# sec-bit/ckb-zkp

Measured on AMD Instinct MI355X. Metric: Groth16 proofs/sec (2^20 constraints, BN256), higher is better.
Workload: dtype u32 limbs (256-bit Montgomery integers); 1 GPU; Groth16 prove, MiMC-chain R1CS, 1048570 constraints (domain 2^20), 1258284 aux, bn254, G1 x4 + G2 x1 MSM + 4 NTT (7 in the reference: evaluation-form key); curve=bn254, log_domain=20, parallelism=independent proofs x1

## Files before the change

### ckb_zkp_amd/csrc/ctx.hpp

```cpp
#pragma once
#include <hip/hip_runtime.h>
#include <stdint.h>

#include <map>
#include <mutex>
#include <memory>
#include <string>
#include <unordered_map>
#include <vector>

#include "../../include/zkp_accel.h"

namespace zkp {

struct HipError {
  hipError_t e;
  const char* what;
  int line;
};

#define ZKP_HIP(call)                                                   \
  do {                                                                  \
    hipError_t _e = (call);                                             \
    if (_e != hipSuccess) throw ::zkp::HipError{_e, #call, __LINE__};   \
  } while (0)

struct StatusError {
  int32_t status;
};
#define ZKP_REQUIRE(cond, status) \
  do {                            \
    if (!(cond)) throw ::zkp::StatusError{(status)}; \
  } while (0)

struct DevBuf {
  void* p = nullptr;
  size_t cap = 0;
  void* get(size_t bytes) {
    if (bytes > cap) {
      if (p) (void)hipFree(p);
      p = nullptr;
      cap = 0;
      size_t want = bytes + (bytes >> 3) + 256;
      hipError_t e = hipMalloc(&p, want);
      if (e != hipSuccess) throw StatusError{ZKP_ERR_OOM};
      cap = want;
    }
    return p;
  }
  template <class T>
  T* as(size_t count) { return reinterpret_cast<T*>(get(count * sizeof(T))); }
  ~DevBuf() {
    if (p) (void)hipFree(p);
  }
  DevBuf() = default;
  DevBuf(const DevBuf&) = delete;
  DevBuf& operator=(const DevBuf&) = delete;
};

struct NttTables {
  int log_n = 0, h = 0;
  uint32_t* w_lo = nullptr;
  uint32_t* w_hi = nullptr;
  uint32_t* wi_lo = nullptr;
  uint32_t* wi_hi = nullptr;
  uint32_t* g_lo = nullptr;
  uint32_t* g_hi = nullptr;
  uint32_t* gi_lo = nullptr;
  uint32_t* gi_hi = nullptr;
  uint32_t* sub_fwd = nullptr;
  uint32_t* sub_inv = nullptr;
  uint32_t* n_inv = nullptr;
  void* block = nullptr;
  uint32_t* full_fwd[8] = {};
  uint32_t* full_inv[8] = {};
  uint32_t* full_g = nullptr;
  uint32_t* full_gi = nullptr;
  uint32_t* g_hi_n = nullptr;
  uint32_t* full_g_n = nullptr;
  std::vector<void*> extra;
};

struct BasesEntry;

struct MsmWorkspace {
  hipStream_t stream = nullptr;
  bool own_stream = false;
  hipEvent_t done = nullptr;
  hipEvent_t sorted = nullptr;
  hipEvent_t l1_done = nullptr;
  uint32_t chain_nb = 0;
  size_t chain_xb = 0;
  hipEvent_t acc_done = nullptr;
  DevBuf keys, vals, keys2, vals2, sort_tmp, offsets, buckets, tmp, out, sched, scan_tmp, scan_tmp2, partial, redo;
};
struct Groth16Timing {
  zkp_groth16_timing t{};
};

}

struct zkp_lane {
  hipStream_t stream = nullptr;
  bool own_stream = true;
  static constexpr int N_WS = 4;
  static constexpr int N_WS_MSM = N_WS;
  zkp::MsmWorkspace ws[N_WS];
  zkp::DevBuf ntt_scratch;
  hipEvent_t ev_fork = nullptr, ev_a = nullptr, ev_b1 = nullptr;
  uint32_t* host_proof = nullptr;
  bool host_tail = false;
  bool busy = false;
};

struct zkp_cfg {
  int lanes = 0;
  int msm_batch_lanes = 1;
  int msm_c = 0, msm_c_g2 = 0;
  long long msm_chunk = (long long)3 << 19;
  double table_budget_gb = 0;
  bool h_lagrange = true, c_fold = true, host_affine = true;
  long long lfold_heavy_cost = 0;
  int multi_exchange = 0;
  int multi_exchange_timeout_ms = 30000;
  int multi_wm_split = -1;
};

struct zkp_ctx {
  int device = 0;
  zkp_cfg cfg;
  std::recursive_mutex mu;
  static constexpr int N_LANES = 8;
  static constexpr int N_WS = zkp_lane::N_WS;
  zkp_lane lanes[N_LANES];
  zkp_lane* cur = &lanes[0];
  int cur_idx = 0;
  hipEvent_t ev0 = nullptr, ev1 = nullptr;
  hipEvent_t ev2 = nullptr, ev3 = nullptr;
  bool profiling = false;
  size_t table_bytes = 0;
  bool msm_defer_reduce = false;
  int msm_acc_into = -1;
  int msm_bucket_ws = -1;
  bool dbg_skip_k8 = false;
  bool batch_mode = false;
  std::map<std::pair<int, int>, zkp::NttTables> ntt_tables;
  zkp::DevBuf ntt_io, poly_tmp, poly_consts, spmv_list;
  zkp::DevBuf msm_scalars, msm_misc, var_bases;
  uint32_t* pinned = nullptr;
  size_t pinned_cap = 0;
  std::unordered_map<uint64_t, std::shared_ptr<zkp::BasesEntry>> bases;
  uint64_t next_handle = 1;
  zkp_groth16_timing last_timing{};
  zkp_marlin_timing last_marlin_timing{};
  std::string last_error;
  std::vector<zkp_ctx*> devs;
  std::map<std::pair<int, int>, std::shared_ptr<void>> var_plans;
  bool tl_on = false;
  std::string tl_tag;
  std::vector<std::pair<std::string, hipEvent_t>> tl;
  void mark(hipStream_t st, const char* what) {
    if (!tl_on) return;
    hipEvent_t e = nullptr;
    if (hipEventCreate(&e) != hipSuccess) return;
    (void)hipEventRecord(e, st);
    tl.emplace_back(tl_tag + what, e);
  }
};
```

### ckb_zkp_amd/csrc/groth16.hip

```cpp
#include <algorithm>
#include <cstdlib>
#include <cstring>
#include <memory>
#include <string>
#include <vector>

#include "field_dev.hpp"
#include "host_field.hpp"
#include "internal.hpp"
#include "msm_vtbl.hpp"

using namespace zkp;

struct DevCsr {
  uint32_t* row_ptr = nullptr;
  uint32_t* col = nullptr;
  uint32_t* coeff = nullptr;
  size_t nnz = 0;
};

struct zkp_groth16_pk {
  int curve = 0;
  uint32_t num_inputs = 0, num_aux = 0, num_constraints = 0;
  int log_n = 0;
// ... 502 lines not shown
        bases_set_sort_flags(ctx, pk->hA, all.data(), all.size());
        bases_set_group(ctx, pk->hA, member.data(), member.size());
        bases_set_filter_bit(ctx, pk->hA, 0);
        if (with_b) bases_set_filter_bit(ctx, pk->hB2, 1);
        bases_set_filter_bit(ctx, pk->hL, 2);
        pk->share_l1 = true;
        pk->b_in_l1 = with_b;
      }
      {
        static const bool on_chain = !(getenv("ZKP_CHAIN_LH") && atoi(getenv("ZKP_CHAIN_LH")) == 0);
        uint64_t iL[5], iH[5];
        bases_info(ctx, pk->hL, iL);
        bases_info(ctx, pk->hH, iH);
        pk->chain_lh = on_chain && iL[0] == iH[0] && iL[2] == 1 && iH[2] == 1 && pk->q_n[3] > 0 && pk->q_n[4] > 0;
      }
      if (getenv("ZKP_DEBUG_MSM"))
        fprintf(stderr, "[groth16] A/L sort sharing: %d (flags differ at %zu of %zu bases), B1/B2: %d, shared level 1: %d\n",
                (int)pk->share_al_sort, differ, fA.size(), (int)pk->share_b_sort, (int)pk->share_l1);
    }
  }
  uint32_t* consts = pk->consts.as<uint32_t>(64);
  if (d->curve == ZKP_BN254) hipLaunchKernelGGL(qap_consts_kernel<Bn254Fr>, dim3(1), dim3(64), 0, ctx->cur->stream, consts, lg);
  else hipLaunchKernelGGL(qap_consts_kernel<Bls381Fr>, dim3(1), dim3(64), 0, ctx->cur->stream, consts, lg);
  ZKP_HIP(hipGetLastError());
  for (int l = 0; l < 2; l++) {
    auto& L = pk->lane[l];
    L.abc.get(3 * pk->N * 32);
    L.S.get((pk->nz + 4) * 32);
    L.results.get(6 * 16 * 24 * 4 + 64);
    L.proof.get(4096);
  }
  ZKP_HIP(hipStreamSynchronize(ctx->cur->stream));
  return pk.release();
}

void groth16_pk_free(zkp_ctx* ctx, zkp_groth16_pk* pk) {
  (void)hipDeviceSynchronize();
  for (auto& PL : pk->lane) {
    if (PL.graph_exec) (void)hipGraphExecDestroy(PL.graph_exec);
    if (PL.graph) (void)hipGraphDestroy(PL.graph);
  }
  for (uint64_t h : {pk->hA, pk->hB1, pk->hB2, pk->hH, pk->hL})
    if (h) bases_drop(ctx, h);
  for (auto& m : pk->m) {
    if (m.row_ptr) (void)hipFree(m.row_ptr);
    if (m.col) (void)hipFree(m.col);
    if (m.coeff) (void)hipFree(m.coeff);
  }
  delete pk;
}

uint64_t groth16_domain_size(zkp_groth16_pk* pk) { return pk->N; }
void groth16_pk_info(zkp_ctx* ctx, zkp_groth16_pk* pk, uint64_t info[8]) {
  for (int i = 0; i < 8; i++) info[i] = 0;
  if (!pk->hA) return;
  uint64_t a[5], b[5];
  bases_info(ctx, pk->hA, a);
  bases_info(ctx, pk->hB2, b);
  info[0] = a[2];
  for (uint64_t h : {pk->hA, pk->hB1, pk->hB2, pk->hH, pk->hL}) {
    uint64_t t[5];
    bases_info(ctx, h, t);
    info[1] += t[4];
  }
  info[2] = a[0];
  info[3] = a[1];
  info[4] = a[3];
  info[5] = b[0];
  info[6] = (pk->share_b_sort ? 1 : 0) | (pk->share_al_sort ? 2 : 0) | (pk->share_l1 ? 4 : 0);
  info[7] = (pk->h_lagrange ? 1 : 0) | (pk->c_folded ? 2 : 0) | (pk->chain_lh ? 4 : 0);
}

template <class P>
static uint32_t* witness_map_dev(zkp_ctx* ctx, zkp_groth16_pk* pk, const uint32_t* z_dev, bool coeffs = true) {
  const uint32_t N = (uint32_t)pk->N;
  uint32_t* a = pk->lane[ctx->cur_idx].abc.as<uint32_t>(3 * pk->N * 8);
  uint32_t* b = a + pk->N * 8;
  uint32_t* c = b + pk->N * 8;
  uint32_t* bufs[3] = {a, b, c};
  hipStream_t st = ctx->cur->stream;
  const int nchain = (!coeffs && pk->c_folded) ? 2 : 3;
  for (int k = 0; k < nchain; k++)
    hipLaunchKernelGGL(csr_eval_kernel<P>, dim3((N + 255) / 256), dim3(256), 0, st, pk->m[k].row_ptr, pk->m[k].col,
                       pk->m[k].coeff, z_dev, pk->num_constraints, N, pk->num_inputs, k == 0 ? 1 : 0, bufs[k]);
  static const bool batch = getenv("ZKP_NTT_BATCH") && atoi(getenv("ZKP_NTT_BATCH")) != 0;
  if (batch) {
    ntt_run_batch(ctx, pk->curve, bufs, nchain, pk->log_n, ZKP_NTT_IFFT);
    ntt_run_batch(ctx, pk->curve, bufs, nchain, pk->log_n, ZKP_NTT_COSET_FFT);
  } else {
    for (int k = 0; k < nchain; k++) {
      if (!ntt_ifft_coset_fft(ctx, pk->curve, bufs[k], pk->log_n)) {
        ntt_run(ctx, pk->curve, bufs[k], pk->log_n, ZKP_NTT_IFFT);
        ntt_run(ctx, pk->curve, bufs[k], pk->log_n, ZKP_NTT_COSET_FFT);
      }
    }
  }
  if (!coeffs) {
    if (pk->c_folded) hipLaunchKernelGGL(qap_pointwise_ab_kernel<P>, dim3((N + 255) / 256), dim3(256), 0, st, a, b, pk->consts.as<uint32_t>(64), N);
    else hipLaunchKernelGGL(qap_pointwise_kernel<P>, dim3((N + 255) / 256), dim3(256), 0, st, a, b, c, pk->consts.as<uint32_t>(64), N);
    ZKP_HIP(hipGetLastError());
    return a;
  }
  if (uint32_t* hq = ntt_qap_coset_ifft(ctx, pk->curve, a, b, c, pk->consts.as<uint32_t>(64), pk->log_n)) {
    ZKP_HIP(hipGetLastError());
    return hq;
  }
  hipLaunchKernelGGL(qap_pointwise_kernel<P>, dim3((N + 255) / 256), dim3(256), 0, st, a, b, c,
                     pk->consts.as<uint32_t>(64), N);
  ntt_run(ctx, pk->curve, a, pk->log_n, ZKP_NTT_COSET_IFFT);
  ZKP_HIP(hipGetLastError());
  return a;
}

void groth16_witness_map(zkp_ctx* ctx, zkp_groth16_pk* pk, const uint64_t* z, uint64_t* h, bool on_device) {
  const uint32_t* zd = reinterpret_cast<const uint32_t*>(z);
  if (!on_device) {
    uint32_t* s = pk->lane[ctx->cur_idx].S.as<uint32_t>((pk->nz + 4) * 8);
    ZKP_HIP(hipMemcpyAsync(s, z, pk->nz * 32, hipMemcpyHostToDevice, ctx->cur->stream));
    zd = s;
  }
  uint32_t* hd = pk->curve == ZKP_BN254 ? witness_map_dev<Bn254Fr>(ctx, pk, zd) : witness_map_dev<Bls381Fr>(ctx, pk, zd);
  ZKP_HIP(hipMemcpyAsync(h, hd, pk->N * 32, on_device ? hipMemcpyDeviceToDevice : hipMemcpyDeviceToHost, ctx->cur->stream));
  if (!on_device) ZKP_HIP(hipStreamSynchronize(ctx->cur->stream));
}

template <class FrP>
static void prove_enqueue_part(zkp_ctx* ctx, zkp_groth16_pk* pk, const uint64_t* z, bool z_on_device, const uint64_t* r,
                               const uint64_t* s, int part, char* partial_out = nullptr, bool latency_plan = false) {
  ZKP_REQUIRE((pk->shard_world > 0) == (partial_out != nullptr), ZKP_ERR_BAD_ARG);
  ZKP_REQUIRE(pk->hA != 0, ZKP_ERR_BAD_ARG);
  zkp_groth16_pk::PerLane& PL = pk->lane[ctx->cur_idx];
  hipStream_t st = ctx->cur->stream;
  const bool prof = ctx->profiling;
  const bool host_tail = ctx->cfg.host_affine && !partial_out;
  zkp_groth16_timing tm{};
  struct ProfEvents {
    hipEvent_t e[4] = {nullptr, nullptr, nullptr, nullptr};
    ~ProfEvents() {
      for (hipEvent_t x : e)
        if (x) (void)hipEventDestroy(x);
    }
  } pev;
  if (prof)
    for (hipEvent_t& x : pev.e) ZKP_HIP(hipEventCreate(&x));
  hipEvent_t &e0 = pev.e[0], &e1 = pev.e[1], &eT0 = pev.e[2], &eT1 = pev.e[3];
  auto tic = [&] { if (prof) ZKP_HIP(hipEventRecord(e0, st)); };
  auto toc = [&](float* dst) {
    if (!prof) return;
    ZKP_HIP(hipEventRecord(e1, st));
    ZKP_HIP(hipEventSynchronize(e1));
    ZKP_HIP(hipEventElapsedTime(dst, e0, e1));
  };
  if (prof) ZKP_HIP(hipEventRecord(eT0, st));
  uint32_t* S = PL.S.as<uint32_t>((pk->nz + 4) * 8);
  uint32_t* rs = PL.proof.as<uint32_t>(1024);
  uint32_t* proof_dev = rs + 16;
  uint32_t* flags_dev = proof_dev + 256;
  if (part & 1) {
    ZKP_HIP(hipMemcpyAsync(S, z, pk->nz * 32, z_on_device ? hipMemcpyDeviceToDevice : hipMemcpyHostToDevice, st));
    ZKP_HIP(hipMemcpyAsync(rs, r, 32, hipMemcpyHostToDevice, st));
    ZKP_HIP(hipMemcpyAsync(rs + 8, s, 32, hipMemcpyHostToDevice, st));
  }
  if (!(part & 2)) return;
  hipLaunchKernelGGL(scalar_tail_kernel<FrP>, dim3(1), dim3(64), 0, st, S + pk->nz * 8, rs);

  const MsmVtbl* v1 = msm_vtbl(pk->curve, 1);
  const MsmVtbl* v2 = msm_vtbl(pk->curve, 2);
  const size_t slot = v2->xyzz_bytes;
  char* res = reinterpret_cast<char*>(PL.results.get(6 * slot));
  const uint64_t* Sd = reinterpret_cast<const uint64_t*>(S);
  bool l_done_in_fan = false, g2_done_in_fan = false, chained = false;
  float acc_ms = 0.f, scan_ms = 0.f;
  uint64_t ent = 0, scan_bytes = 0, scan_runs = 0;
  static const bool single_stream = getenv("ZKP_SINGLE_STREAM") && atoi(getenv("ZKP_SINGLE_STREAM")) != 0;
  const bool fan = !prof && !single_stream;
  uint32_t* h = nullptr;
  auto run = [&](int idx, uint64_t handle, const uint64_t* sc, size_t n, int w, int sort_src = -1, int l1_src = -1) {
    float ms = 0.f, ms_sc = 0.f;
    uint64_t e = 0;
    static const char* const names[5] = {"A", "B1", "B2", "H", "L"};
    ctx->tl_tag = names[idx];
    tic();
#ifdef ZKP_ABLATION
    static const int skip_k8 = [] { const char* e = getenv("ZKP_DEBUG_SKIP_K8_MASK"); return e ? (int)strtol(e, nullptr, 0) : 0; }();
    ctx->dbg_skip_k8 = ((skip_k8 >> idx) & 1) && ctx->batch_mode;
#endif
    msm_run(ctx, handle, 0, sc, n, true, nullptr, res + idx * slot, prof ? &ms : nullptr, &e, fan ? w : 0,
            fan ? sort_src : -1, prof ? &ms_sc : nullptr, fan ? l1_src : -1);
    ctx->dbg_skip_k8 = false;
    toc(&tm.ms_msm[idx]);
    acc_ms += ms;
    ent += e;
    tm.ms_msm_acc[idx] = ms;
    tm.msm_entries[idx] = e;
    if (ms_sc > 0.f) {
      scan_ms += ms_sc;
      scan_bytes += 2 * 32 * (uint64_t)n + 8 * e;
      scan_runs += 1;
    }
    tm.msm_accumulate_launches += 1;
  };
  ctx->tl_tag.clear();
  ctx->mark(st, "start");
  if (fan) {
    ZKP_HIP(hipEventRecord(ctx->cur->ev_fork, st));
    for (int w = 1; w < zkp_ctx::N_WS; w++) ZKP_HIP(hipStreamWaitEvent(ctx->cur->ws[w].stream, ctx->cur->ev_fork, 0));
    static const bool wm_first = !(getenv("ZKP_WM_FIRST") && atoi(getenv("ZKP_WM_FIRST")) == 0);
    if (wm_first) {
      h = witness_map_dev<FrP>(ctx, pk, S, !pk->h_lagrange);
      ctx->mark(st, "wm");
    }
    static const bool l_own = !(getenv("ZKP_L_OWN_STREAM") && atoi(getenv("ZKP_L_OWN_STREAM")) == 0);
    static const int lat_env = [] { const char* e = getenv("ZKP_LATENCY_PLAN"); return e ? atoi(e) : -1; }();
    (void)latency_plan;
    const bool lat = lat_env >= 0 ? lat_env != 0 : true;
    if (lat) {
      const int l1 = pk->share_l1 ? 1 : -1;
      const bool b_l1 = pk->share_l1 && pk->b_in_l1;
      if (!b_l1) run(2, pk->hB2, Sd + 4 * pk->q_lo[2], pk->q_n[2], 2);
      run(0, pk->hA, Sd + 4 * pk->q_lo[0], pk->q_n[0], 1);
      ZKP_HIP(hipEventRecord(ctx->cur->ev_a, ctx->cur->ws[1].stream));
      if (b_l1) run(2, pk->hB2, Sd + 4 * pk->q_lo[2], pk->q_n[2], 2, -1, l1);
      static const bool g2_early = !(getenv("ZKP_G2_EARLY") && atoi(getenv("ZKP_G2_EARLY")) == 0);
      if (!partial_out && g2_early && !host_tail) {
        v2->assemble_g2(ctx->cur->ws[2].stream, res, slot, proof_dev, flags_dev, 2 * v1->fN);
        g2_done_in_fan = true;
      }
      run(1, pk->hB1, Sd + 4 * pk->q_lo[1], pk->q_n[1], 3, pk->share_b_sort ? 2 : -1);
      ctx->msm_defer_reduce = chained = pk->chain_lh;
      run(4, pk->hL, Sd + 4 * pk->q_lo[4], pk->q_n[4], 1, pk->share_al_sort ? 1 : -1, l1);
      if (!partial_out) {
        ZKP_HIP(hipStreamWaitEvent(ctx->cur->ws[3].stream, ctx->cur->ev_a, 0));
        v1->assemble_g1_part1(ctx->cur->ws[3].stream, res, slot, rs, host_tail ? nullptr : proof_dev, flags_dev);
        ctx->tl_tag.clear();
        ctx->mark(ctx->cur->ws[3].stream, "part1");
      }
    } else {
    run(2, pk->hB2, Sd + 4 * pk->q_lo[2], pk->q_n[2], 2);
    run(0, pk->hA, Sd + 4 * pk->q_lo[0], pk->q_n[0], 1);
    run(1, pk->hB1, Sd + 4 * pk->q_lo[1], pk->q_n[1], 1, pk->share_b_sort ? 2 : -1);
    if (l_own) run(4, pk->hL, Sd + 4 * pk->q_lo[4], pk->q_n[4], 3, pk->share_al_sort && pk->share_b_sort ? 1 : -1);
    ZKP_HIP(hipEventRecord(ctx->cur->ev_b1, ctx->cur->ws[1].stream));
    if (!partial_out) {
      ZKP_HIP(hipStreamWaitEvent(ctx->cur->ws[3].stream, ctx->cur->ev_b1, 0));
      v1->assemble_g1_part1(ctx->cur->ws[3].stream, res, slot, rs, host_tail ? nullptr : proof_dev, flags_dev);
    }
    }
    l_done_in_fan = lat || l_own;
  }
  tic();
  if (!h) h = witness_map_dev<FrP>(ctx, pk, S, !pk->h_lagrange);
  toc(&tm.ms_witness_map);
  if (!fan) {
    run(0, pk->hA, Sd + 4 * pk->q_lo[0], pk->q_n[0], 0);
    run(1, pk->hB1, Sd + 4 * pk->q_lo[1], pk->q_n[1], 0);
    run(2, pk->hB2, Sd + 4 * pk->q_lo[2], pk->q_n[2], 0);
  }
  if (chained) ctx->msm_acc_into = 1;
  run(3, pk->hH, reinterpret_cast<const uint64_t*>(h) + 4 * pk->q_lo[3], pk->q_n[3], 0);
  if (!(fan && l_done_in_fan)) run(4, pk->hL, Sd + 4 * pk->q_lo[4], pk->q_n[4], 0);
  if (fan) {
    for (int w = 1; w < zkp_ctx::N_WS; w++) {
      ZKP_HIP(hipEventRecord(ctx->cur->ws[w].done, ctx->cur->ws[w].stream));
      ZKP_HIP(hipStreamWaitEvent(st, ctx->cur->ws[w].done, 0));
    }
  }
  tm.ms_msm_accumulate = acc_ms;
  tm.msm_points = ent;
  tm.ms_msm_scan = scan_ms;
  tm.msm_scan_bytes = scan_bytes;
  tm.msm_scan_launches = scan_runs;
  if (partial_out) {
    ZKP_HIP(hipMemcpyAsync(partial_out, res, 5 * slot, hipMemcpyDeviceToDevice, st));
    ZKP_HIP(hipGetLastError());
    if (prof) {
      ZKP_HIP(hipEventRecord(eT1, st));
      ZKP_HIP(hipStreamSynchronize(st));
      ZKP_HIP(hipEventElapsedTime(&tm.ms_total, eT0, eT1));
      ctx->last_timing = tm;
    }
    return;
  }

  tic();
  if (!fan) v1->assemble_g1_part1(st, res, slot, rs, host_tail ? nullptr : proof_dev, flags_dev);
  v1->assemble_g1_part2(st, res, slot, host_tail ? nullptr : proof_dev, flags_dev, 2 * v1->fN + 2 * v2->fN);
  if (!g2_done_in_fan && !host_tail) v2->assemble_g2(st, res, slot, proof_dev, flags_dev, 2 * v1->fN);
  ZKP_HIP(hipGetLastError());
  toc(&tm.ms_assemble);
  const size_t proof_words = 4 * (size_t)v1->fN + 2 * (size_t)v2->fN;
  if (host_tail) {
    uint32_t* hp = ctx->cur->host_proof;
    ZKP_HIP(hipMemcpyAsync(hp, res, 16 * (size_t)v1->fN, hipMemcpyDeviceToHost, st));
    ZKP_HIP(hipMemcpyAsync(hp + 4 * v1->fN, res + 2 * slot, 16 * (size_t)v2->fN, hipMemcpyDeviceToHost, st));
    ZKP_HIP(hipMemcpyAsync(hp + 4 * v1->fN + 4 * v2->fN, res + 5 * slot, 16 * (size_t)v1->fN, hipMemcpyDeviceToHost, st));
  } else {
    ZKP_HIP(hipMemcpyAsync(ctx->cur->host_proof, proof_dev, proof_words * 4, hipMemcpyDeviceToHost, st));
    ZKP_HIP(hipMemcpyAsync(ctx->cur->host_proof + 256, flags_dev, 12, hipMemcpyDeviceToHost, st));
  }
  ctx->tl_tag.clear();
  ctx->mark(st, "copied");
  ctx->cur->host_tail = host_tail;
  ctx->cur->busy = true;
  if (prof) {
    ZKP_HIP(hipEventRecord(eT1, st));
    ZKP_HIP(hipStreamSynchronize(st));
    ZKP_HIP(hipEventElapsedTime(&tm.ms_total, eT0, eT1));
    ctx->last_timing = tm;
  }
}

static std::vector<const void*> lane_signature(zkp_ctx* ctx, zkp_groth16_pk* pk) {
  std::vector<const void*> sig;
  zkp_lane* L = ctx->cur;
  zkp_groth16_pk::PerLane& PL = pk->lane[ctx->cur_idx];
  for (DevBuf* b : {&PL.abc, &PL.S, &PL.results, &PL.proof, &L->ntt_scratch}) sig.push_back(b->p);
  for (int w = 0; w < zkp_lane::N_WS; w++) {
    MsmWorkspace& ws = L->ws[w];
    for (DevBuf* b : {&ws.keys, &ws.vals, &ws.keys2, &ws.vals2, &ws.sort_tmp, &ws.offsets, &ws.buckets, &ws.tmp, &ws.out,
                      &ws.sched, &ws.scan_tmp, &ws.scan_tmp2, &ws.partial, &ws.redo})
      sig.push_back(b->p);
  }
  sig.push_back(pk);
  return sig;
}

template <class FrP>
static void prove_enqueue(zkp_ctx* ctx, zkp_groth16_pk* pk, const uint64_t* z, bool z_on_device, const uint64_t* r,
                          const uint64_t* s, bool latency_plan = false) {
  static const bool graph_on = getenv("ZKP_GRAPH") && atoi(getenv("ZKP_GRAPH")) != 0;
  static const bool single_stream = getenv("ZKP_SINGLE_STREAM") && atoi(getenv("ZKP_SINGLE_STREAM")) != 0;
  if (!graph_on || ctx->profiling || single_stream) {
    prove_enqueue_part<FrP>(ctx, pk, z, z_on_device, r, s, 3, nullptr, latency_plan);
    return;
  }
  zkp_groth16_pk::PerLane& PL = pk->lane[ctx->cur_idx];
  hipStream_t st = ctx->cur->stream;
  if (PL.graph_state == 2 && PL.sig == lane_signature(ctx, pk)) {
    prove_enqueue_part<FrP>(ctx, pk, z, z_on_device, r, s, 1);
    ZKP_HIP(hipGraphLaunch(PL.graph_exec, st));
    ctx->cur->busy = true;
    return;
  }
  if (PL.graph_state == 2) {
    (void)hipGraphExecDestroy(PL.graph_exec);
    (void)hipGraphDestroy(PL.graph);
    PL.graph_exec = nullptr;
    PL.graph = nullptr;
    PL.graph_state = 0;
  }
  if (PL.graph_state == 1 && PL.sig == lane_signature(ctx, pk)) {
    prove_enqueue_part<FrP>(ctx, pk, z, z_on_device, r, s, 1);
    ZKP_HIP(hipStreamBeginCapture(st, hipStreamCaptureModeRelaxed));
    try {
      prove_enqueue_part<FrP>(ctx, pk, z, z_on_device, r, s, 2);
    } catch (...) {
      hipGraph_t g = nullptr;
      (void)hipStreamEndCapture(st, &g);
      if (g) (void)hipGraphDestroy(g);
      throw;
    }
    ZKP_HIP(hipStreamEndCapture(st, &PL.graph));
    ZKP_HIP(hipGraphInstantiate(&PL.graph_exec, PL.graph, nullptr, nullptr, 0));
    PL.graph_state = 2;
    ZKP_HIP(hipGraphLaunch(PL.graph_exec, st));
    ctx->cur->busy = true;
    return;
  }
  prove_enqueue_part<FrP>(ctx, pk, z, z_on_device, r, s, 3);
  PL.sig = lane_signature(ctx, pk);
  PL.graph_state = 1;
}

static void prove_finish(zkp_ctx* ctx, zkp_groth16_pk* pk, uint64_t* proof_out, uint8_t* inf_out) {
  const MsmVtbl* v1 = msm_vtbl(pk->curve, 1);
  const MsmVtbl* v2 = msm_vtbl(pk->curve, 2);
  const size_t proof_words = 4 * (size_t)v1->fN + 2 * (size_t)v2->fN;
  ZKP_HIP(hipStreamSynchronize(ctx->cur->stream));
  if (!ctx->tl.empty()) {
    std::string line = "[zkp timeline ms]";
    for (auto& m : ctx->tl) {
      float ms = 0.f;
      (void)hipEventSynchronize(m.second);
      (void)hipEventElapsedTime(&ms, ctx->tl[0].second, m.second);
      char buf[64];
      snprintf(buf, sizeof buf, " %s=%.2f", m.first.c_str(), ms);
      line += buf;
      if (&m != &ctx->tl[0]) (void)hipEventDestroy(m.second);
    }
    (void)hipEventDestroy(ctx->tl[0].second);
    ctx->tl.clear();
    fprintf(stderr, "%s\n", line.c_str());
  }
  if (ctx->cur->host_tail) {
    const hostf::HostField Fq = hostf::fq_field(pk->curve);
    const uint32_t* hp = ctx->cur->host_proof;
    hostf::groth16_points_into_affine(Fq, hp, hp + 4 * v1->fN, hp + 4 * v1->fN + 4 * v2->fN,
                                      reinterpret_cast<uint32_t*>(proof_out), inf_out);
  } else {
    memcpy(proof_out, ctx->cur->host_proof, proof_words * 4);
    for (int i = 0; i < 3; i++) inf_out[i] = (uint8_t)ctx->cur->host_proof[256 + i];
  }
  ctx->cur->busy = false;
}

void groth16_assemble(zkp_ctx* ctx, int curve, const uint64_t* sums, const uint64_t* r, const uint64_t* s,
                      uint64_t* proof_out, uint8_t* inf_out) {
  const MsmVtbl* v1 = msm_vtbl(curve, 1);
  const MsmVtbl* v2 = msm_vtbl(curve, 2);
  hipStream_t st = ctx->cur->stream;
  const size_t slot = v2->xyzz_bytes;
  const size_t j1 = 3 * (size_t)v1->fN, j2 = 3 * (size_t)v2->fN;
  const size_t in_words = 4 * j1 + j2;
  uint32_t* buf = ctx->msm_misc.as<uint32_t>(in_words + 16 + 6 * slot / 4 + 256 + 16);
  uint32_t* jac = buf;
  uint32_t* rs = jac + in_words;
  char* res = reinterpret_cast<char*>(rs + 16);
  uint32_t* proof_dev = reinterpret_cast<uint32_t*>(res + 6 * slot);
  uint32_t* flags_dev = proof_dev + 240;
  ZKP_HIP(hipMemcpyAsync(jac, sums, in_words * 4, hipMemcpyHostToDevice, st));
  ZKP_HIP(hipMemcpyAsync(rs, r, 32, hipMemcpyHostToDevice, st));
  ZKP_HIP(hipMemcpyAsync(rs + 8, s, 32, hipMemcpyHostToDevice, st));
  const size_t off[5] = {0, j1, 2 * j1, 2 * j1 + j2, 3 * j1 + j2};
  for (int i = 0; i < 5; i++) (i == 2 ? v2 : v1)->from_jacobian(st, jac + off[i], res + i * slot);
  v1->assemble_g1_part1(st, res, slot, rs, proof_dev, flags_dev);
  v1->assemble_g1_part2(st, res, slot, proof_dev, flags_dev, 2 * v1->fN + 2 * v2->fN);
  v2->assemble_g2(st, res, slot, proof_dev, flags_dev, 2 * v1->fN);
  ZKP_HIP(hipGetLastError());
  const size_t proof_words = 4 * (size_t)v1->fN + 2 * (size_t)v2->fN;
  uint32_t flags_host[4] = {0, 0, 0, 0};
  ZKP_HIP(hipMemcpyAsync(proof_out, proof_dev, proof_words * 4, hipMemcpyDeviceToHost, st));
  ZKP_HIP(hipMemcpyAsync(flags_host, flags_dev, 12, hipMemcpyDeviceToHost, st));
  ZKP_HIP(hipStreamSynchronize(st));
  for (int i = 0; i < 3; i++) inf_out[i] = (uint8_t)flags_host[i];
}

size_t groth16_partials_bytes(int curve) { return 5 * msm_vtbl(curve, 2)->xyzz_bytes; }

void groth16_prove_partials(zkp_ctx* ctx, zkp_groth16_pk* pk, const uint64_t* z_dev, const uint64_t* r, const uint64_t* s,
                            void* out_dev) {
  ZKP_REQUIRE(pk->shard_world > 0, ZKP_ERR_BAD_ARG);
  ctx->cur = &ctx->lanes[0];
  ctx->cur_idx = 0;
  if (pk->curve == ZKP_BN254) prove_enqueue_part<Bn254Fr>(ctx, pk, z_dev, true, r, s, 3, (char*)out_dev, true);
  else prove_enqueue_part<Bls381Fr>(ctx, pk, z_dev, true, r, s, 3, (char*)out_dev, true);
  ZKP_HIP(hipStreamSynchronize(ctx->cur->stream));
}

void groth16_fold_assemble(zkp_ctx* ctx, int curve, const void* gathered_dev, int world, const uint64_t* r,
                           const uint64_t* s, uint64_t* proof_out, uint8_t* inf_out) {
  ZKP_REQUIRE(world >= 1, ZKP_ERR_BAD_ARG);
  const MsmVtbl* v1 = msm_vtbl(curve, 1);
  const MsmVtbl* v2 = msm_vtbl(curve, 2);
  hipStream_t st = ctx->cur->stream;
  const size_t slot = v2->xyzz_bytes;
  uint32_t* buf = ctx->msm_misc.as<uint32_t>(16 + 6 * slot / 4 + 256 + 16);
  uint32_t* rs = buf;
  char* res = reinterpret_cast<char*>(rs + 16);
  uint32_t* proof_dev = reinterpret_cast<uint32_t*>(res + 6 * slot);
  uint32_t* flags_dev = proof_dev + 240;
  ZKP_HIP(hipMemcpyAsync(rs, r, 32, hipMemcpyHostToDevice, st));
  ZKP_HIP(hipMemcpyAsync(rs + 8, s, 32, hipMemcpyHostToDevice, st));
  v1->fold_slots(st, (const char*)gathered_dev, 5 * slot, world, slot, 0x1b, res);
  v2->fold_slots(st, (const char*)gathered_dev, 5 * slot, world, slot, 0x04, res);
  v1->assemble_g1_part1(st, res, slot, rs, proof_dev, flags_dev);
  v1->assemble_g1_part2(st, res, slot, proof_dev, flags_dev, 2 * v1->fN + 2 * v2->fN);
  v2->assemble_g2(st, res, slot, proof_dev, flags_dev, 2 * v1->fN);
  ZKP_HIP(hipGetLastError());
  const size_t proof_words = 4 * (size_t)v1->fN + 2 * (size_t)v2->fN;
  uint32_t flags_host[4] = {0, 0, 0, 0};
  ZKP_HIP(hipMemcpyAsync(proof_out, proof_dev, proof_words * 4, hipMemcpyDeviceToHost, st));
  ZKP_HIP(hipMemcpyAsync(flags_host, flags_dev, 12, hipMemcpyDeviceToHost, st));
  ZKP_HIP(hipStreamSynchronize(st));
  for (int i = 0; i < 3; i++) inf_out[i] = (uint8_t)flags_host[i];
}

void groth16_prove(zkp_ctx* ctx, zkp_groth16_pk* pk, const uint64_t* z, bool z_on_device, const uint64_t* r,
                   const uint64_t* s, uint64_t* proof_out, uint8_t* inf_out) {
  ZKP_REQUIRE(pk->shard_world == 0, ZKP_ERR_BAD_ARG);
  ctx->cur = &ctx->lanes[0];
  ctx->cur_idx = 0;
  static const bool timeline = getenv("ZKP_TIMELINE") && atoi(getenv("ZKP_TIMELINE")) != 0;
  ctx->tl_on = timeline && !ctx->profiling;
  if (pk->curve == ZKP_BN254) prove_enqueue<Bn254Fr>(ctx, pk, z, z_on_device, r, s, true);
  else prove_enqueue<Bls381Fr>(ctx, pk, z, z_on_device, r, s, true);
  ctx->tl_on = false;
  prove_finish(ctx, pk, proof_out, inf_out);
}

void groth16_prove_batch(zkp_ctx* ctx, zkp_groth16_pk* pk, size_t n, const uint64_t* const* z_dev, const uint64_t* r,
                         const uint64_t* s, uint64_t* proofs_out, uint8_t* inf_out, bool z_on_device) {
  const MsmVtbl* v1 = msm_vtbl(pk->curve, 1);
  const MsmVtbl* v2 = msm_vtbl(pk->curve, 2);
  const size_t pw64 = (4 * (size_t)v1->fN + 2 * (size_t)v2->fN) / 2;
  const bool prof = ctx->profiling;
  ZKP_REQUIRE(pk->shard_world == 0, ZKP_ERR_BAD_ARG);
  size_t pending[zkp_ctx::N_LANES] = {};
  const int lanes_default = pk->log_n <= 22 ? 8 : 4;
  const int nl = std::max(1, std::min(ctx->cfg.lanes > 0 ? ctx->cfg.lanes : lanes_default, (int)zkp_ctx::N_LANES));
  auto select = [&](int l) {
    ctx->cur = &ctx->lanes[l];
    ctx->cur_idx = l;
  };
  struct BatchMode {
    zkp_ctx* c;
    ~BatchMode() { c->batch_mode = false; }
  } batch_mode{ctx};
  ctx->batch_mode = n > 1 && !prof;
  try {
    if (ctx->batch_mode) {
      std::vector<uint64_t> scratch_proof(pw64 + 8);
      uint8_t scratch_inf[4];
      bool any = false;
      for (int l = 0; l < nl; l++) {
        if (pk->lane[l].warmed) continue;
        select(l);
        if (pk->curve == ZKP_BN254) prove_enqueue<Bn254Fr>(ctx, pk, z_dev[0], z_on_device, r, s);
        else prove_enqueue<Bls381Fr>(ctx, pk, z_dev[0], z_on_device, r, s);
        pk->lane[l].warmed = true;
        any = true;
      }
      if (any)
        for (int l = 0; l < nl; l++) {
          select(l);
          if (ctx->cur->busy) prove_finish(ctx, pk, scratch_proof.data(), scratch_inf);
        }
    }
    for (size_t i = 0; i < n; i++) {
      const int l = prof ? 0 : (int)(i % nl);
      select(l);
      if (ctx->cur->busy) prove_finish(ctx, pk, proofs_out + pending[l] * pw64, inf_out + pending[l] * 3);
      if (pk->curve == ZKP_BN254) prove_enqueue<Bn254Fr>(ctx, pk, z_dev[i], z_on_device, r + 4 * i, s + 4 * i);
      else prove_enqueue<Bls381Fr>(ctx, pk, z_dev[i], z_on_device, r + 4 * i, s + 4 * i);
      pending[l] = i;
    }
    for (int l = 0; l < zkp_ctx::N_LANES; l++) {
      select(l);
      if (ctx->cur->busy) prove_finish(ctx, pk, proofs_out + pending[l] * pw64, inf_out + pending[l] * 3);
    }
  } catch (...) {
    (void)hipDeviceSynchronize();
    for (auto& L : ctx->lanes) L.busy = false;
    select(0);
    throw;
  }
  select(0);
}

}
#include <dlfcn.h>

#include <chrono>
#include <condition_variable>
#include <mutex>
#include <string>

#include <thread>
struct zkp_groth16_pk_multi {
  int mode = 0, curve = 0;
  std::vector<zkp_groth16_pk*> pk;
  std::vector<hipEvent_t> ev_chain, ev_done, ev_h_read;
  hipEvent_t ev_h = nullptr;
  void* gathered = nullptr;
  std::vector<void*> gathered_all;
  std::vector<void*> partial;
  int exchange = 0;
  bool exchange_fallback = false;
  int rccl_ranks = 0;
  int split_choice = -1;
  int calls = 0;
  double ms_variant[2] = {0.0, 0.0};
};
namespace zkp {

namespace {
struct RcclApi {
  struct Fns {
    void* lib = nullptr;
    int (*CommInitAll)(void**, int, const int*) = nullptr;
    int (*CommDestroy)(void*) = nullptr;
    int (*CommAbort)(void*) = nullptr;
    int (*GroupStart)() = nullptr;
    int (*GroupEnd)() = nullptr;
    int (*AllGather)(const void*, void*, size_t, int, void*, hipStream_t) = nullptr;
  };
  struct Attempt {
    std::mutex m;
    std::condition_variable cv;
    bool done = false, ok = false, abandoned = false;
    Fns f;
    std::vector<void*> comms;
    std::string why;
  };
  Fns f;
  std::mutex mu;
  std::map<std::vector<int>, std::vector<void*>> comms_of;
  bool unusable = false, watchdog_fired = false;
  std::string why;

  static void bring_up(std::shared_ptr<Attempt> at, std::vector<int> ids, int timeout_ms) {
    const char* hang = getenv("ZKP_DEBUG_RCCL_HANG");
    Fns f;
    std::vector<void*> comms(ids.size(), nullptr);
    std::string why;
    bool ok = false;
    do {
      for (const char* name : {"librccl.so", "librccl.so.1"})
        if ((f.lib = dlopen(name, RTLD_NOW | RTLD_LOCAL))) break;
      if (!f.lib) { why = "librccl.so not loadable"; break; }
      f.CommInitAll = reinterpret_cast<decltype(f.CommInitAll)>(dlsym(f.lib, "ncclCommInitAll"));
      f.CommDestroy = reinterpret_cast<decltype(f.CommDestroy)>(dlsym(f.lib, "ncclCommDestroy"));
      f.CommAbort = reinterpret_cast<decltype(f.CommAbort)>(dlsym(f.lib, "ncclCommAbort"));
      f.GroupStart = reinterpret_cast<decltype(f.GroupStart)>(dlsym(f.lib, "ncclGroupStart"));
      f.GroupEnd = reinterpret_cast<decltype(f.GroupEnd)>(dlsym(f.lib, "ncclGroupEnd"));
      f.AllGather = reinterpret_cast<decltype(f.AllGather)>(dlsym(f.lib, "ncclAllGather"));
      if (!f.CommInitAll || !f.CommDestroy || !f.GroupStart || !f.GroupEnd || !f.AllGather) { why = "librccl.so lacks a symbol"; break; }
      if (hang && !strcmp(hang, "init")) std::this_thread::sleep_for(std::chrono::hours(24));
      if (f.CommInitAll(comms.data(), (int)ids.size(), ids.data()) != 0) { why = "ncclCommInitAll failed"; comms.clear(); break; }
      const int n = (int)ids.size();
      std::vector<hipStream_t> st(n, nullptr);
      std::vector<void*> snd(n, nullptr), rcv(n, nullptr);
      bool issued = true;
      for (int k = 0; k < n && issued; k++)
        issued = hipSetDevice(ids[k]) == hipSuccess && hipStreamCreateWithFlags(&st[k], hipStreamNonBlocking) == hipSuccess &&
                 hipMalloc(&snd[k], 64) == hipSuccess && hipMalloc(&rcv[k], 64 * (size_t)n) == hipSuccess &&
                 hipMemsetAsync(snd[k], k + 1, 64, st[k]) == hipSuccess;
      if (issued) {
        issued = f.GroupStart() == 0;
        for (int k = 0; k < n && issued; k++)
          issued = hipSetDevice(ids[k]) == hipSuccess && f.AllGather(snd[k], rcv[k], 64,  1, comms[k], st[k]) == 0;
        issued = f.GroupEnd() == 0 && issued;
      }
      bool drained = false, right = true;
      if (issued) {
        const auto deadline = std::chrono::steady_clock::now() + std::chrono::milliseconds(timeout_ms);
        while (!drained && std::chrono::steady_clock::now() < deadline) {
          drained = !(hang && !strcmp(hang, "probe"));
          for (int k = 0; k < n && drained; k++) drained = hipStreamQuery(st[k]) == hipSuccess;
          if (!drained) std::this_thread::sleep_for(std::chrono::milliseconds(2));
        }
        if (drained) {
          std::vector<uint8_t> got(64 * (size_t)n);
          for (int k = 0; k < n && right; k++) {
            right = hipSetDevice(ids[k]) == hipSuccess && hipMemcpy(got.data(), rcv[k], got.size(), hipMemcpyDeviceToHost) == hipSuccess;
            for (int j = 0; j < n && right; j++) right = got[64 * (size_t)j] == (uint8_t)(j + 1) && got[64 * (size_t)j + 63] == (uint8_t)(j + 1);
          }
        }
      }
      if (!issued || !drained || !right) {
        why = !issued ? "the probe all-gather could not be enqueued" : !drained ? "the probe all-gather did not complete within " + std::to_string(timeout_ms) + " ms"
                      : "the probe all-gather returned wrong bytes";
        for (void* c : comms)
          if (c) (void)(f.CommAbort ? f.CommAbort(c) : f.CommDestroy(c));
        comms.clear();
        if (!drained) break;
      }
      for (int k = 0; k < n; k++) {
        (void)hipSetDevice(ids[k]);
        if (st[k]) (void)hipStreamDestroy(st[k]);
        if (snd[k]) (void)hipFree(snd[k]);
        if (rcv[k]) (void)hipFree(rcv[k]);
      }
      ok = issued && drained && right;
    } while (false);
    std::lock_guard<std::mutex> lk(at->m);
    if (at->abandoned) {
      for (void* c : comms)
        if (c && f.CommAbort) (void)f.CommAbort(c);
      return;
    }
    at->f = f;
    at->comms = ok ? comms : std::vector<void*>();
    at->ok = ok;
    at->why = why;
    at->done = true;
    at->cv.notify_all();
  }

  const std::vector<void*>* ready(const std::vector<zkp_ctx*>& devs, int timeout_ms) {
    if (unusable) return nullptr;
    std::vector<int> ids;
    for (zkp_ctx* d : devs) ids.push_back(d->device);
    if (auto it = comms_of.find(ids); it != comms_of.end()) return &it->second;
    for (size_t i = 0; i < ids.size(); i++)
      for (size_t j = i + 1; j < ids.size(); j++)
        if (ids[i] == ids[j]) { why = "duplicate device ids"; return nullptr; }
    timeout_ms = std::max(1, timeout_ms);
    auto at = std::make_shared<Attempt>();
    std::thread(bring_up, at, ids, timeout_ms).detach();
    std::unique_lock<std::mutex> lk(at->m);
    const bool back = at->cv.wait_for(lk, std::chrono::milliseconds(2 * (long long)timeout_ms + 2000), [&] { return at->done; });
    if (!back) {
      at->abandoned = true;
      unusable = watchdog_fired = true;
      why = "RCCL bring-up (ncclCommInitAll + probe all-gather) did not return within " + std::to_string(2 * (long long)timeout_ms + 2000) + " ms";
// ... 348 lines not shown
```

Before: 137.6 proofs/s.

## Rotate input and tail stages onto workspace streams in batch mode

In batch mode with fan-out, the input copies and scalar tail kernel now go on workspace stream 1. The final assembly and device-to-host proof copies go on workspace stream 3 instead of the lane's main stream, and prove_finish synchronizes on that tail stream. The aim is to let the next proof's work on the main stream start without queuing behind the previous proof's input and tail stages, so consecutive proofs overlap more. It adds cross-stream event dependencies, which risk ordering hazards if a buffer is reused across proofs.

```diff
diff --git a/ckb_zkp_amd/csrc/ctx.hpp b/ckb_zkp_amd/csrc/ctx.hpp
--- a/ckb_zkp_amd/csrc/ctx.hpp
+++ b/ckb_zkp_amd/csrc/ctx.hpp
@@ -111,6 +111,7 @@
   uint32_t* host_proof = nullptr;
   bool host_tail = false;
   bool busy = false;
+  hipStream_t tail = nullptr;
 };
 
 struct zkp_cfg {
diff --git a/ckb_zkp_amd/csrc/groth16.hip b/ckb_zkp_amd/csrc/groth16.hip
--- a/ckb_zkp_amd/csrc/groth16.hip
+++ b/ckb_zkp_amd/csrc/groth16.hip
@@ -678,17 +678,24 @@
     ZKP_HIP(hipEventElapsedTime(dst, e0, e1));
   };
   if (prof) ZKP_HIP(hipEventRecord(eT0, st));
+  static const bool single_stream = getenv("ZKP_SINGLE_STREAM") && atoi(getenv("ZKP_SINGLE_STREAM")) != 0;
+  const bool fan = !prof && !single_stream;
+  static const bool batch_plan_on = !(getenv("ZKP_BATCH_PLAN") && atoi(getenv("ZKP_BATCH_PLAN")) == 0);
+  static const bool graph_on = getenv("ZKP_GRAPH") && atoi(getenv("ZKP_GRAPH")) != 0;
+  const bool shared_q = batch_plan_on && ctx->batch_mode && fan && !partial_out && !graph_on && part == 3;
+  hipStream_t st_in = shared_q ? ctx->cur->ws[1].stream : st;
+  hipStream_t st_tail = shared_q ? ctx->cur->ws[3].stream : st;
   uint32_t* S = PL.S.as<uint32_t>((pk->nz + 4) * 8);
   uint32_t* rs = PL.proof.as<uint32_t>(1024);
   uint32_t* proof_dev = rs + 16;
   uint32_t* flags_dev = proof_dev + 256;
   if (part & 1) {
-    ZKP_HIP(hipMemcpyAsync(S, z, pk->nz * 32, z_on_device ? hipMemcpyDeviceToDevice : hipMemcpyHostToDevice, st));
-    ZKP_HIP(hipMemcpyAsync(rs, r, 32, hipMemcpyHostToDevice, st));
-    ZKP_HIP(hipMemcpyAsync(rs + 8, s, 32, hipMemcpyHostToDevice, st));
+    ZKP_HIP(hipMemcpyAsync(S, z, pk->nz * 32, z_on_device ? hipMemcpyDeviceToDevice : hipMemcpyHostToDevice, st_in));
+    ZKP_HIP(hipMemcpyAsync(rs, r, 32, hipMemcpyHostToDevice, st_in));
+    ZKP_HIP(hipMemcpyAsync(rs + 8, s, 32, hipMemcpyHostToDevice, st_in));
   }
   if (!(part & 2)) return;
-  hipLaunchKernelGGL(scalar_tail_kernel<FrP>, dim3(1), dim3(64), 0, st, S + pk->nz * 8, rs);
+  hipLaunchKernelGGL(scalar_tail_kernel<FrP>, dim3(1), dim3(64), 0, st_in, S + pk->nz * 8, rs);
 
   const MsmVtbl* v1 = msm_vtbl(pk->curve, 1);
   const MsmVtbl* v2 = msm_vtbl(pk->curve, 2);
@@ -698,8 +705,6 @@
   bool l_done_in_fan = false, g2_done_in_fan = false, chained = false;
   float acc_ms = 0.f, scan_ms = 0.f;
   uint64_t ent = 0, scan_bytes = 0, scan_runs = 0;
-  static const bool single_stream = getenv("ZKP_SINGLE_STREAM") && atoi(getenv("ZKP_SINGLE_STREAM")) != 0;
-  const bool fan = !prof && !single_stream;
   uint32_t* h = nullptr;
   auto run = [&](int idx, uint64_t handle, const uint64_t* sc, size_t n, int w, int sort_src = -1, int l1_src = -1) {
     float ms = 0.f, ms_sc = 0.f;
@@ -729,8 +734,11 @@
   ctx->tl_tag.clear();
   ctx->mark(st, "start");
   if (fan) {
-    ZKP_HIP(hipEventRecord(ctx->cur->ev_fork, st));
-    for (int w = 1; w < zkp_ctx::N_WS; w++) ZKP_HIP(hipStreamWaitEvent(ctx->cur->ws[w].stream, ctx->cur->ev_fork, 0));
+    ZKP_HIP(hipEventRecord(ctx->cur->ev_fork, st_in));
+    for (int w = 0; w < zkp_ctx::N_WS; w++) {
+      hipStream_t sw = w == 0 ? st : ctx->cur->ws[w].stream;
+      if (sw != st_in) ZKP_HIP(hipStreamWaitEvent(sw, ctx->cur->ev_fork, 0));
+    }
     static const bool wm_first = !(getenv("ZKP_WM_FIRST") && atoi(getenv("ZKP_WM_FIRST")) == 0);
     if (wm_first) {
       h = witness_map_dev<FrP>(ctx, pk, S, !pk->h_lagrange);
@@ -786,9 +794,11 @@
   run(3, pk->hH, reinterpret_cast<const uint64_t*>(h) + 4 * pk->q_lo[3], pk->q_n[3], 0);
   if (!(fan && l_done_in_fan)) run(4, pk->hL, Sd + 4 * pk->q_lo[4], pk->q_n[4], 0);
   if (fan) {
-    for (int w = 1; w < zkp_ctx::N_WS; w++) {
-      ZKP_HIP(hipEventRecord(ctx->cur->ws[w].done, ctx->cur->ws[w].stream));
-      ZKP_HIP(hipStreamWaitEvent(st, ctx->cur->ws[w].done, 0));
+    for (int w = 0; w < zkp_ctx::N_WS; w++) {
+      hipStream_t sw = w == 0 ? st : ctx->cur->ws[w].stream;
+      if (sw == st_tail) continue;
+      ZKP_HIP(hipEventRecord(ctx->cur->ws[w].done, sw));
+      ZKP_HIP(hipStreamWaitEvent(st_tail, ctx->cur->ws[w].done, 0));
     }
   }
   tm.ms_msm_accumulate = acc_ms;
@@ -810,22 +820,23 @@
 
   tic();
   if (!fan) v1->assemble_g1_part1(st, res, slot, rs, host_tail ? nullptr : proof_dev, flags_dev);
-  v1->assemble_g1_part2(st, res, slot, host_tail ? nullptr : proof_dev, flags_dev, 2 * v1->fN + 2 * v2->fN);
-  if (!g2_done_in_fan && !host_tail) v2->assemble_g2(st, res, slot, proof_dev, flags_dev, 2 * v1->fN);
+  v1->assemble_g1_part2(st_tail, res, slot, host_tail ? nullptr : proof_dev, flags_dev, 2 * v1->fN + 2 * v2->fN);
+  if (!g2_done_in_fan && !host_tail) v2->assemble_g2(st_tail, res, slot, proof_dev, flags_dev, 2 * v1->fN);
   ZKP_HIP(hipGetLastError());
   toc(&tm.ms_assemble);
   const size_t proof_words = 4 * (size_t)v1->fN + 2 * (size_t)v2->fN;
   if (host_tail) {
     uint32_t* hp = ctx->cur->host_proof;
-    ZKP_HIP(hipMemcpyAsync(hp, res, 16 * (size_t)v1->fN, hipMemcpyDeviceToHost, st));
-    ZKP_HIP(hipMemcpyAsync(hp + 4 * v1->fN, res + 2 * slot, 16 * (size_t)v2->fN, hipMemcpyDeviceToHost, st));
-    ZKP_HIP(hipMemcpyAsync(hp + 4 * v1->fN + 4 * v2->fN, res + 5 * slot, 16 * (size_t)v1->fN, hipMemcpyDeviceToHost, st));
+    ZKP_HIP(hipMemcpyAsync(hp, res, 16 * (size_t)v1->fN, hipMemcpyDeviceToHost, st_tail));
+    ZKP_HIP(hipMemcpyAsync(hp + 4 * v1->fN, res + 2 * slot, 16 * (size_t)v2->fN, hipMemcpyDeviceToHost, st_tail));
+    ZKP_HIP(hipMemcpyAsync(hp + 4 * v1->fN + 4 * v2->fN, res + 5 * slot, 16 * (size_t)v1->fN, hipMemcpyDeviceToHost, st_tail));
   } else {
-    ZKP_HIP(hipMemcpyAsync(ctx->cur->host_proof, proof_dev, proof_words * 4, hipMemcpyDeviceToHost, st));
-    ZKP_HIP(hipMemcpyAsync(ctx->cur->host_proof + 256, flags_dev, 12, hipMemcpyDeviceToHost, st));
+    ZKP_HIP(hipMemcpyAsync(ctx->cur->host_proof, proof_dev, proof_words * 4, hipMemcpyDeviceToHost, st_tail));
+    ZKP_HIP(hipMemcpyAsync(ctx->cur->host_proof + 256, flags_dev, 12, hipMemcpyDeviceToHost, st_tail));
   }
   ctx->tl_tag.clear();
-  ctx->mark(st, "copied");
+  ctx->mark(st_tail, "copied");
+  ctx->cur->tail = st_tail;
   ctx->cur->host_tail = host_tail;
   ctx->cur->busy = true;
   if (prof) {
@@ -902,7 +913,9 @@
   const MsmVtbl* v1 = msm_vtbl(pk->curve, 1);
   const MsmVtbl* v2 = msm_vtbl(pk->curve, 2);
   const size_t proof_words = 4 * (size_t)v1->fN + 2 * (size_t)v2->fN;
-  ZKP_HIP(hipStreamSynchronize(ctx->cur->stream));
+  hipStream_t tail = ctx->cur->tail ? ctx->cur->tail : ctx->cur->stream;
+  ctx->cur->tail = nullptr;
+  ZKP_HIP(hipStreamSynchronize(tail));
   if (!ctx->tl.empty()) {
     std::string line = "[zkp timeline ms]";
     for (auto& m : ctx->tl) {
@@ -1066,7 +1079,10 @@
     }
   } catch (...) {
     (void)hipDeviceSynchronize();
-    for (auto& L : ctx->lanes) L.busy = false;
+    for (auto& L : ctx->lanes) {
+      L.busy = false;
+      L.tail = nullptr;
+    }
     select(0);
     throw;
   }
```

Result: slower. 135.5 proofs/s (-1.5%).
